# BurryChen/lv_slam

Hardware: AMD Instinct MI355X
Metric: NDT registrations/sec (64k-pt Velodyne pairs) (higher is better)
Workload: dtype f32 terms, f64 accumulation

## Files before the change

lv_slam_amd/csrc/ndt_build.hpp:

```cpp
#pragma once
#include "ndt_types.hpp"
#include "ndt_math.hpp"

__device__ __forceinline__ unsigned mm_enc_max(int ord) { return (unsigned)ord ^ 0x80000000u; }
__device__ __forceinline__ unsigned mm_enc_min(int ord) { return ~((unsigned)ord ^ 0x80000000u); }
__device__ __forceinline__ int mm_dec_max(unsigned e) { return (int)(e ^ 0x80000000u); }
__device__ __forceinline__ int mm_dec_min(unsigned e) { return (int)(~e ^ 0x80000000u); }

#define MM_ILP 3
struct __attribute__((packed, aligned(4))) MmQuad { float v[4]; };
__global__ void __launch_bounds__(256) k_minmax(const float* __restrict__ tgt, size_t pitch, const int* __restrict__ cnt, unsigned* mm) {
  const int b = blockIdx.y;
  const int n = cnt[b];
  const float* X = tgt + (size_t)b * 3 * pitch;
  int mn[3] = {INT_MAX, INT_MAX, INT_MAX}, mx[3] = {INT_MIN, INT_MIN, INT_MIN};
  auto take = [&](const float x, const float y, const float z) {
    if (!finite3(x, y, z)) return;
    const int ox = f2ord(x), oy = f2ord(y), oz = f2ord(z);
    mn[0] = min(mn[0], ox); mx[0] = max(mx[0], ox);
    mn[1] = min(mn[1], oy); mx[1] = max(mx[1], oy);
    mn[2] = min(mn[2], oz); mx[2] = max(mx[2], oz);
  };
  const int stride = (int)(gridDim.x * blockDim.x) * 4;
  for (int i0 = (int)(blockIdx.x * blockDim.x + threadIdx.x) * 4; i0 < n; i0 += stride * MM_ILP) {
// ... 158 lines not shown
  const int nw = gd[b].nwords;
  const int lane = threadIdx.x & 63, wv = threadIdx.x >> 6;
  unsigned base = 0;
  for (int w0 = 0; w0 < nw; w0 += RANK_THREADS * RANK_ROWS) {
    const int wbase = w0 + wv * 64 * RANK_ROWS;
    unsigned c[RANK_ROWS], ex[RANK_ROWS], run = 0;
#pragma unroll
    for (int u = 0; u < RANK_ROWS; u++) { const int w = wbase + u * 64 + lane; c[u] = (w < nw) ? (unsigned)__popcll(W[w].bits) : 0u; }
#pragma unroll
    for (int u = 0; u < RANK_ROWS; u++) {
      unsigned inc = c[u];
#pragma unroll
      for (int o = 1; o < 64; o <<= 1) { const unsigned t = __shfl_up(inc, o); if (lane >= o) inc += t; }
      ex[u] = run + inc - c[u];
      run += __shfl(inc, 63);
    }
    if (lane == 0) wtot[wv] = run;
    __syncthreads();
    if (wv == 0) {
      const unsigned v = lane < RANK_WAVES ? wtot[lane] : 0u;
      unsigned inc = v;
#pragma unroll
      for (int o = 1; o < RANK_WAVES; o <<= 1) { const unsigned t = __shfl_up(inc, o); if (lane >= o) inc += t; }
      if (lane < RANK_WAVES) wtot[lane] = inc - v;
      if (lane == RANK_WAVES - 1) wtot[16] = inc;
    }
    __syncthreads();
    const unsigned off = base + wtot[wv];
#pragma unroll
    for (int u = 0; u < RANK_ROWS; u++) { const int w = wbase + u * 64 + lane; if (w < nw) W[w].prefix = off + ex[u]; }
    base += wtot[16];
    __syncthreads();
  }
  if (threadIdx.x == 0) gd[b].n_voxels = (int)base;
  unsigned hbase = 0;
  for (unsigned q0 = 0; q0 < n_slices; q0 += RANK_THREADS) {
    const unsigned q = q0 + threadIdx.x;
    const unsigned c = q < n_slices ? head_cnt[(size_t)b * n_slices + q] : 0u;
    unsigned tot;
    const unsigned ex = block_exscan<RANK_THREADS>(c, &tot, wtot);
    const unsigned* H = heads + ((size_t)b * n_slices + q) * slice_cap;
    unsigned* S = seg_start + gd[b].rec_off + hbase + ex;
    for (unsigned k = 0; k < c; k++) S[k] = H[k];
    hbase += tot;
  }
}

__global__ void __launch_bounds__(256) k_sorted_points(const float* __restrict__ tgt, size_t pitch, const unsigned* __restrict__ vals, float4* __restrict__ sorted,
                                                        int nx, int n_targets) {
  int b, bx;
  if (!xcd_map(nx, n_targets, bx, b)) return;
  const float* X = tgt + (size_t)b * 3 * pitch;
  const unsigned* V = vals + (size_t)b * pitch;
  float4* P = sorted + (size_t)b * pitch;
  const size_t i0 = ((size_t)bx * 256 + threadIdx.x);
  const size_t stride = (size_t)nx * 256;
  for (size_t i = i0; i < pitch; i += stride * RUN_ILP) {
    unsigned v[RUN_ILP];
    float4 q[RUN_ILP];
#pragma unroll
    for (int u = 0; u < RUN_ILP; u++) { const size_t j = i + u * stride; v[u] = j < pitch ? V[j] : 0u; }
#pragma unroll
    for (int u = 0; u < RUN_ILP; u++) { const unsigned k = v[u] < pitch ? v[u] : 0u; q[u] = make_float4(X[k], X[pitch + k], X[2 * pitch + k], 0.f); }
#pragma unroll
    for (int u = 0; u < RUN_ILP; u++) { const size_t j = i + u * stride; if (j < pitch) P[j] = q[u]; }
  }
}

#ifdef NDT_TIMELINE
__device__ unsigned long long g_ltl[16];
#define LTL_DECL unsigned long long ltl[12] = {0, 0, 0, 0, 0, 0, 0, 0, 0, 0, 0, 0}; unsigned long long ltl_last = __builtin_readcyclecounter(); const unsigned long long ltl_t0 = ltl_last
#define LTL_STAMP(k) do { __builtin_amdgcn_sched_barrier(0); const unsigned long long t_ = __builtin_readcyclecounter(); ltl[k] += t_ - ltl_last; ltl_last = t_; __builtin_amdgcn_sched_barrier(0); } while (0)
#define LTL_COUNT(k, v) do { ltl[k] += (unsigned long long)(v); } while (0)
#define LTL_FLUSH() do { ltl[10] = 1; ltl[11] = __builtin_readcyclecounter() - ltl_t0; if ((threadIdx.x & 63) == 0 && (blockIdx.x % 24) == (threadIdx.x >> 6) * 5) for (int k_ = 0; k_ < 12; k_++) atomicAdd(&g_ltl[k_], ltl[k_]); } while (0)
#define LTL_ARRIVED1(a) asm volatile("" : "+v"(a))
#else
#define LTL_DECL do {} while (0)
#define LTL_STAMP(k) do {} while (0)
#define LTL_COUNT(k, v) do {} while (0)
#define LTL_FLUSH() do {} while (0)
#define LTL_ARRIVED1(a) do {} while (0)
#endif
#define LS_WAVES 4
template <typename KeyT, bool CENT, bool SORTED = false>
__global__ void __launch_bounds__(64 * LS_WAVES) k_leafsum(const float* __restrict__ tgt, size_t pitch,
                                                           const KeyT* __restrict__ keys, const unsigned* __restrict__ vals ,
                                                           const GridDesc* __restrict__ gd, const unsigned* __restrict__ seg_start,
                                                           double* sums, int* vox_idx, int* vox_n, int cb, float* cent,
                                                           int nx, int n_targets) {
  __shared__ double term[LS_WAVES][64][9];
  __shared__ float termf[CENT ? LS_WAVES : 1][64][3];
  int b, bx;
  if (!xcd_map(nx, n_targets, bx, b)) return;
  const GridDesc& g = gd[b];
  const int lane = threadIdx.x & 63, wv = threadIdx.x >> 6;
  const KeyT* K = keys + (size_t)b * pitch;
  const unsigned* V = vals + (size_t)b * pitch;
  const float* X = tgt + (size_t)b * 3 * pitch;
  const int id0 = bx * LS_WAVES + wv, idstep = nx * LS_WAVES;
  size_t start_next = id0 < g.n_voxels ? seg_start[g.rec_off + id0] : 0;
  LTL_DECL;
  for (int id = id0; id < g.n_voxels; id += idstep) {
    LTL_COUNT(9, 1);
    const size_t start = start_next;
    if (id + idstep < g.n_voxels) start_next = seg_start[g.rec_off + id + idstep];
    double acc = (lane == 3 || lane == 6 || lane == 8) ? 1.0 : 0.0;
    float accf = 0.f;
    int cnt = 0;
    KeyT key = 0;
    for (size_t j0 = start;; j0 += 64) {
      const size_t j = j0 + lane;
      const bool inb = j < pitch;
      const KeyT kj = inb ? K[j] : (KeyT)0;
      float4 pj = make_float4(0.f, 0.f, 0.f, 0.f);
      unsigned pi = 0u;
      if (SORTED) { if (inb) pj = reinterpret_cast<const float4*>(vals)[(size_t)b * pitch + j]; }
      else pi = inb ? V[j] : 0u;
#ifdef NDT_TIMELINE
      { KeyT kq = kj; LTL_ARRIVED1(kq); LTL_ARRIVED1(pi); LTL_ARRIVED1(pj.x); }
      LTL_STAMP(0);
      LTL_COUNT(8, 1);
#endif
      if (j0 == start) key = __shfl(kj, 0);
      const bool in = inb && kj == key;
      const int m = (int)__popcll(__ballot(in));
      if (in) {
        float fx = SORTED ? pj.x : X[pi], fy = SORTED ? pj.y : X[pitch + pi], fz = SORTED ? pj.z : X[2 * pitch + pi];
        LTL_ARRIVED1(fx); LTL_ARRIVED1(fy); LTL_ARRIVED1(fz);
        LTL_STAMP(1);
        const double x = (double)fx, y = (double)fy, z = (double)fz;
        double* t = term[wv][lane];
        t[0] = x; t[1] = y; t[2] = z;
        t[3] = x * x; t[4] = x * y; t[5] = x * z; t[6] = y * y; t[7] = y * z; t[8] = z * z;
        if (CENT) { termf[wv][lane][0] = fx; termf[wv][lane][1] = fy; termf[wv][lane][2] = fz; }
      }
      __builtin_amdgcn_wave_barrier();
      LTL_STAMP(2);
      if (lane < 9) {
        int l = 0;
        for (; l + 8 <= m; l += 8) {
          double t[8];
#pragma unroll
          for (int u = 0; u < 8; u++) t[u] = term[wv][l + u][lane];
#pragma unroll
          for (int u = 0; u < 8; u++) acc += t[u];
        }
        for (; l < m; l++) acc += term[wv][l][lane];
      } else if (CENT && lane < 12) {
        for (int l = 0; l < m; l++) accf += termf[wv][l][lane - 9];
      }
      __builtin_amdgcn_wave_barrier();
      LTL_STAMP(3);
      cnt += m;
      if (m < 64) break;
    }
    if (lane < 9) sums[(size_t)(g.rec_off + id) * 9 + lane] = acc;
    else if (CENT && lane < 12) cent[(size_t)(g.rec_off + id) * 3 + (lane - 9)] = accf / (float)cnt;
    if (lane == 0) {
      vox_idx[g.rec_off + id] = (int)((unsigned)key & ((1u << cb) - 1u));
      vox_n[g.rec_off + id] = cnt;
    }
    LTL_STAMP(4);
  }
  LTL_FLUSH();
}

#ifndef LS_TREE_LEAVES
#define LS_TREE_LEAVES 1
#endif
__global__ void __launch_bounds__(64 * LS_WAVES) k_leafsum_tree(const float* __restrict__ tgt, size_t pitch, const unsigned* __restrict__ keys, const unsigned* __restrict__ vals,
                                                                const GridDesc* __restrict__ gd, const unsigned* __restrict__ seg_start,
                                                                double* sums, int* vox_idx, int* vox_n, int cb, int nx, int n_targets) {
  int b, bx;
  if (!xcd_map(nx, n_targets, bx, b)) return;
  const GridDesc& g = gd[b];
  const int lane = threadIdx.x & 63, wv = threadIdx.x >> 6;
  const unsigned* K = keys + (size_t)b * pitch;
  const unsigned* V = vals + (size_t)b * pitch;
  const float* X = tgt + (size_t)b * 3 * pitch;
  constexpr int NL = LS_TREE_LEAVES;
  const int id0 = bx * LS_WAVES + wv, idstep = nx * LS_WAVES;
  const int nv = g.n_voxels;
  for (int idb = id0; idb < nv; idb += NL * idstep) {
    size_t start[NL];
    bool have[NL];
#pragma unroll
    for (int u = 0; u < NL; u++) { const int id = idb + u * idstep; have[u] = id < nv; start[u] = have[u] ? seg_start[g.rec_off + id] : 0; }
    double a[NL][9];
    int cnt[NL];
    unsigned key[NL];
    bool more[NL];
#pragma unroll
    for (int u = 0; u < NL; u++) {
#pragma unroll
      for (int k = 0; k < 9; k++) a[u][k] = 0.0;
      cnt[u] = 0; key[u] = 0u; more[u] = have[u];
    }
    for (int chunk = 0;; chunk++) {
      bool any = false;
#pragma unroll
      for (int u = 0; u < NL; u++) any = any || more[u];
      if (!any) break;
      unsigned kj[NL], pi[NL];
      bool inb[NL];
#pragma unroll
      for (int u = 0; u < NL; u++) {
        const size_t j = start[u] + (size_t)chunk * 64 + lane;
        inb[u] = more[u] && j < pitch;
        kj[u] = inb[u] ? K[j] : 0u;
        pi[u] = inb[u] ? V[j] : 0u;
      }
      float fx[NL], fy[NL], fz[NL];
      bool in[NL];
#pragma unroll
      for (int u = 0; u < NL; u++) {
        if (chunk == 0) key[u] = __shfl(kj[u], 0);
        in[u] = inb[u] && kj[u] == key[u];
        fx[u] = fy[u] = fz[u] = 0.f;
        if (in[u]) { fx[u] = X[pi[u]]; fy[u] = X[pitch + pi[u]]; fz[u] = X[2 * pitch + pi[u]]; }
      }
#pragma unroll
      for (int u = 0; u < NL; u++) {
        const int m = (int)__popcll(__ballot(in[u]));
        if (in[u]) {
          const double x = (double)fx[u], y = (double)fy[u], z = (double)fz[u];
          a[u][0] += x; a[u][1] += y; a[u][2] += z;
          a[u][3] += x * x; a[u][4] += x * y; a[u][5] += x * z; a[u][6] += y * y; a[u][7] += y * z; a[u][8] += z * z;
        }
        cnt[u] += m;
        more[u] = more[u] && m == 64;
      }
    }
    typedef unsigned int u2v __attribute__((ext_vector_type(2)));
#pragma unroll
    for (int u = 0; u < NL; u++) {
      if (!have[u]) continue;
      const int id = idb + u * idstep;
      double p1[5], p2[3];
#pragma unroll
      for (int i = 0; i < 5; i++) {
        const double x = a[u][i], v = (i + 5 < 9) ? a[u][i + 5] : 0.0;
        const u2v lo = __builtin_amdgcn_permlane32_swap((unsigned)__double2loint(x), (unsigned)__double2loint(v), false, false);
        const u2v hi = __builtin_amdgcn_permlane32_swap((unsigned)__double2hiint(x), (unsigned)__double2hiint(v), false, false);
        p1[i] = __hiloint2double((int)hi.x, (int)lo.x) + __hiloint2double((int)hi.y, (int)lo.y);
      }
#pragma unroll
      for (int i = 0; i < 3; i++) {
        const double x = p1[i], v = (i + 3 < 5) ? p1[i + 3] : 0.0;
        const u2v lo = __builtin_amdgcn_permlane16_swap((unsigned)__double2loint(x), (unsigned)__double2loint(v), false, false);
        const u2v hi = __builtin_amdgcn_permlane16_swap((unsigned)__double2hiint(x), (unsigned)__double2hiint(v), false, false);
        double w = __hiloint2double((int)hi.x, (int)lo.x) + __hiloint2double((int)hi.y, (int)lo.y);
#pragma unroll
        for (int o = 8; o > 0; o >>= 1) w += __shfl_xor(w, o);
        p2[i] = w;
      }
      if ((lane & 15) == 0) {
        const int row = lane >> 4, base = 3 * (row & 1) + 5 * (row >> 1), nrow = (row & 1) ? ((row >> 1) ? 1 : 2) : 3;
        double* o = sums + (size_t)(g.rec_off + id) * 9;
#pragma unroll
        for (int i = 0; i < 3; i++) if (i < nrow) { const int k = base + i; o[k] = p2[i] + ((k == 3 || k == 6 || k == 8) ? 1.0 : 0.0); }
      }
      if (lane == 0) {
        vox_idx[g.rec_off + id] = (int)(key[u] & ((1u << cb) - 1u));
        vox_n[g.rec_off + id] = cnt[u];
      }
    }
  }
}

__global__ void __launch_bounds__(256) k_voxels(const GridDesc* __restrict__ gd, const double* __restrict__ sums,
                                                 VoxelRec* recs, int* vox_n, double eig_mult, int pca, double* icov64, int* kd_weight,
                                                 VoxelRecF* recs_fast ) {
  const int b = blockIdx.y;
  const GridDesc& g = gd[b];
  const int id = blockIdx.x * blockDim.x + threadIdx.x;
  if (id >= g.n_voxels) return;
  const double* A = sums + (size_t)(g.rec_off + id) * 9;
  const double S[3] = {A[0], A[1], A[2]};
  const double C[9] = {A[3], A[4], A[5], A[4], A[6], A[7], A[5], A[7], A[8]};
  const int cnt = vox_n[g.rec_off + id];
  const double dn = (double)cnt;
  double mu[3] = {S[0] / dn, S[1] / dn, S[2] / dn};
  double cov[9];
  for (int a = 0; a < 3; a++)
    for (int c = 0; c < 3; c++) cov[a * 3 + c] = (C[a * 3 + c] - 2 * (S[a] * mu[c])) / dn + mu[a] * mu[c];
  const double f = (dn - 1.0) / dn;
  for (int a = 0; a < 9; a++) cov[a] *= f;
  double ev[3], Vm[9];
  ndtm::eigen_sym3(cov, ev, Vm);
  VoxelRec r;
  r.mean[0] = mu[0]; r.mean[1] = mu[1]; r.mean[2] = mu[2];
  for (int a = 0; a < 9; a++) r.icov[a] = 0.f;
  r.weight = 1;
  int n_out = cnt, kd_w = 0;
  if (ev[0] < 0 || ev[1] < 0 || ev[2] <= 0) {
    n_out = -1;
    r.weight = VOX_DEAD;
    if (icov64) for (int a = 0; a < 9; a++) icov64[(size_t)(g.rec_off + id) * 9 + a] = 0.0;
  } else {
    const double minev = eig_mult * ev[2];
    if (ev[0] < minev) {
      ev[0] = minev;
      if (ev[1] < minev) ev[1] = minev;
      double VD[9], Vi[9];
      for (int a = 0; a < 3; a++) for (int c = 0; c < 3; c++) VD[a * 3 + c] = Vm[a * 3 + c] * ev[c];
      ndtm::mat3_inverse(Vm, Vi);
      ndtm::mat3_mul(VD, Vi, cov);
    }
    if (pca) {
      double s0 = sqrt(ev[0]), s1 = sqrt(ev[1]), s2 = sqrt(ev[2]);
      double f0 = (s2 - s1) / s2, f1 = (s1 - s0) / s2, f2 = s0 / s2;
      int label = 1;
      double fm = f0;
      if (f1 > fm) { fm = f1; label = 2; }
      if (f2 > fm) { label = 3; }
      double scale = (label == 2) ? 1.25 : ((label == 1) ? 0.75 : 1.0);
      double d2d = scale * sqrt((mu[0] * mu[0] + mu[1] * mu[1]) + mu[2] * mu[2]);
      r.weight = (int)d2d;
      kd_w = r.weight;
    }
    double ic[9];
    ndtm::mat3_inverse(cov, ic);
    bool bad = false;
    for (int a = 0; a < 9; a++) { if (!isfinite(ic[a])) bad = true; r.icov[a] = (float)ic[a]; }
    if (bad) { n_out = -1; r.weight = VOX_DEAD; }
    if (icov64) for (int a = 0; a < 9; a++) icov64[(size_t)(g.rec_off + id) * 9 + a] = ic[a];
  }
  recs[g.rec_off + id] = r;
  vox_n[g.rec_off + id] = n_out;
  if (recs_fast) {
    VoxelRecF f;
    for (int a = 0; a < 3; a++) { f.mh[a] = (float)r.mean[a]; f.ml[a] = (float)(r.mean[a] - (double)f.mh[a]); }
    f.c[0] = r.icov[0]; f.c[1] = 0.5f * (r.icov[1] + r.icov[3]); f.c[2] = 0.5f * (r.icov[2] + r.icov[6]);
    f.c[3] = r.icov[4]; f.c[4] = 0.5f * (r.icov[5] + r.icov[7]); f.c[5] = r.icov[8];
    f.pad_[0] = f.pad_[1] = f.pad_[2] = 0.f;
    f.weight = r.weight;
    recs_fast[g.rec_off + id] = f;
  }
  if (kd_weight) kd_weight[g.rec_off + id] = kd_w;
}
```

lv_slam_amd/csrc/ndt_engine.hpp:

```cpp
#pragma once

struct mi355ndt_handle;
struct EngineDel { void operator()(mi355ndt_handle* e) const { (void)mi355ndt_destroy(e); } };

struct StreamCtx {
  long long batch_id = -1; int n_pairs = 0;
  bool busy = false;
  bool redo = false;
  bool done_sync = false;
  long long launch = -1;
  DevBuf<int> d_in; PinBuf<int> h_in; unsigned* h_in_dev = nullptr;
  PinBuf<mi355ndt_result> h_res; mi355ndt_result* d_res_map = nullptr;
  std::vector<float> guesses;
  PoseRecord* d_pose = nullptr; int pose_cap = 0, pose_base = 0, pose_stride = 1;
  std::unique_ptr<mi355ndt_handle, EngineDel> e;
};
struct StreamState {
  static constexpr int EV = 16;
  bool sync_only = false, drop_carry = true;
  int nctx = 0, max_pairs = 0, items = 0, ring_cap = 0, thresh = 0;
  bool thresh_given = false;
  size_t max_tgt = 0, max_src = 0;
  int plan_cb = 0; size_t plan_words = 0;
  void* pose_next = nullptr; size_t pose_cap_next = 0; int pose_base_next = 0, pose_stride_next = 1;
  long long next_id = 0, launches = 0, counted = 0;
  long long recovered_upto = -1;
  DevBuf<AsyncCtl> d_ctl;
  DevBuf<int> d_ring;
  DevBuf<CtxStat> d_stat;
  HipStream build_stream; int reserve_wg = 0, launch_slots = 0;
  bool lean = false;
  bool reserve_given = false;
  int last_reserve = 0, last_slots = 0;
  HipEvent ev_built[ASYNC_MAX_CTX], ev_launched[EV], ev_prepared[EV]; bool prep_first = true;
  PinBuf<volatile StreamStatus> h_status; StreamStatus* d_status = nullptr;
  StreamCtx ctx[ASYNC_MAX_CTX];
};

struct VoxelScratch {
  DevBuf<float> in, x, out;
  DevBuf<unsigned char> keep;
  DevBuf<unsigned> keys, vals;
  DevBuf<unsigned> hist, offs, tmp;
  DevBuf<int> flag, pos;
  DevBuf<int> mm, cnt, aabb, stat;
  DevBuf<PfGrid> grid; DevBuf<McBox> box;
  DevBuf<unsigned char> tab; PinBuf<unsigned char> h_tab;
  DevBuf<double> part; PinBuf<double> h_part;
  PinBuf<int> h_ret;
  bool pending = false;
};

struct CloudIndex {
  static constexpr int NO_INDEX = -1;
  DevBuf<unsigned char> blob; int status = NO_INDEX; int n_fin = 0;
};

struct GicpCache {
  DevBuf<double> cov;
  int k = -1; double eps = 0.0;
};
struct GicpSide {
  DevBuf<float> rows_own; size_t n = 0, pitch = 0;
  int kf_id = -1; bool set = false;
  CloudIndex index; GicpCache cache;
};

struct mi355ndt_handle {
  int device = 0;
  HipStream own_stream;
  hipStream_t stream = nullptr;
  mi355ndt_params prm;
  std::string err;

  int n_pairs = 0, cap_pairs = 0;
  size_t tgt_pitch = 0, src_pitch = 0;
  size_t own_tgt_pitch = 0, own_src_pitch = 0;
  int own_tgt_pairs = 0, own_src_pairs = 0;
  DevBuf<float> d_tgt_own, d_src_own;
  const float *d_tgt = nullptr, *d_src = nullptr;
  DevBuf<int> d_tgt_cnt_own, d_src_cnt_own;
  int *d_tgt_cnt = nullptr, *d_src_cnt = nullptr;
  std::vector<int> h_tgt_cnt, h_src_cnt;
  std::vector<int> up_tgt_cnt, up_src_cnt;
  bool have_target = false, have_source = false;
  GridsBuilt built{};
  bool aligned_once = false;

  unsigned* d_minmax = nullptr;
  DevBuf<GridDesc> d_grid;
  DevBuf<unsigned> d_nwords, d_word_off;
  DevBuf<unsigned> d_keys_a, d_keys_b;
  DevBuf<unsigned> d_vals_a, d_vals_b;
  DevBuf<BitWord> d_words;
  size_t recs_per_pair = 0;
  DevBuf<VoxelRec> d_recs; DevBuf<int> d_vox_idx, d_vox_n;
  DevBuf<unsigned> d_seg_start; DevBuf<double> d_sums;
  DevBuf<unsigned> d_heads, d_head_cnt;
  DevBuf<float> d_cent; DevBuf<double> d_icov64;
  DevBuf<int> d_kdw;
  DevBuf<float4> d_sorted; bool leaf_sorted = false;
  DevBuf<unsigned> d_rs_hist, d_rs_offs;
  DevBuf<double> d_fit;
  DevBuf<BitWord> d_fwords; DevBuf<unsigned> d_fruns;
  DevBuf<int> d_fit_items; DevBuf<float> d_fit_T;
  DevBuf<float> d_pf_out; int pf_count = 0; size_t pf_pitch = 0;
  CloudIndex ol_index; DevBuf<float> d_ol_dist; PinBuf<float> h_ol_dist;
  int ol_cell_mm = 100;
  int pf_group = 0;
  VoxelScratch vs;
  struct Keyframe {
    DevBuf<float> rows; size_t n = 0, pitch = 0; int ch = 3;
    CloudIndex index;
    GicpCache gicp;
  };
  std::map<int, Keyframe> keyframes;
  int kf_next_id = 0;
  int kff_cell_mm = 100;
  struct Gicp {
    mi355ndt_gicp_params prm{20, 1e-3, 2e-3, 5e-4, 200, 20, 5.0};
    GicpSide side[2];
    DevBuf<int> idx, m; DevBuf<double> maha, part; DevBuf<float> moved;
    PinBuf<double> h_rec; double* d_rec = nullptr;
    bool have_corr = false, have_final = false; int n_matched = 0;
    float final_cm[16] = {1,0,0,0, 0,1,0,0, 0,0,1,0, 0,0,0,1};
  } gicp;
  struct GicpBatch {
    struct Slot {
      GicpSide side;
      DevBuf<int> idx; DevBuf<double> maha, part;
      bool have_final = false; float final_cm[16];
    };
    std::vector<Slot> slot;
    DevBuf<int> m;
    PinBuf<double> h_rec; double* d_rec = nullptr;
    PinBuf<GcSlot> h_tab; DevBuf<GcSlot> d_tab;
    int rounds = 0; std::vector<int> requests;
  } gicp_batch;
  struct IcpWork {
    DevBuf<float> W, d2; DevBuf<int> idx; DevBuf<double> part;
    size_t n = 0, pitch = 0;
    bool have_final = false; IcpRun run;
  };
  struct Icp {
    mi355ndt_icp_params prm{0.0, 10, -DBL_MAX, 1.3407807929942596e154, 3, 0};
    GicpSide side[2];
    IcpWork work;
    DevBuf<int> m; DevBuf<float> moved;
    PinBuf<double> h_rec; double* d_rec = nullptr;
  } icp;
  struct IcpBatch {
    struct Slot { GicpSide side; IcpWork work; };
    std::vector<Slot> slot;
    DevBuf<int> m;
    PinBuf<double> h_rec; double* d_rec = nullptr;
    PinBuf<IcpSlot> h_tab; DevBuf<IcpSlot> d_tab;
    int rounds = 0; std::vector<int> requests;
  } icp_batch;
  float last_final[16] = {1,0,0,0, 0,1,0,0, 0,0,1,0, 0,0,0,1};
  PinBuf<unsigned> h_pin_u;

  DevBuf<PairState> d_state;
  DevBuf<double> d_partials;
  int chunks_per_pair = 0;
  int rows_per_pair = 0, pts_per_chunk = CHUNK_PTS;
  int items_per_pair = 0;
  bool async_force = false;
  bool async_align = true;
  int score_only_last = 1;
  DevBuf<int> d_ring; DevBuf<unsigned> d_arrived; DevBuf<AsyncCtl> d_actl;
  PinBuf<AsyncCtl> h_pin_actl;
  DevBuf<AsyncTab> d_atab;
  unsigned debug_abort_pos = 0xFFFFFFFFu;
  unsigned debug_ring_mask = 0xFFu;
  int sweep_waves = 0;
  int last_async_wpe = 0, last_async_grid = 0;
  int arith = 0;
  DevBuf<VoxelRecF> d_recs_fast;
  int pose_model = 0;
  int ndt_class = 0;
  DevBuf<double> d_pcl_rows;
  DevBuf<float> d_euler_rows;
  int f32_sum_order = 0;
  double gauss_last[3] = {0, 0, 0};
// ... 144 lines not shown
```

lv_slam_amd/csrc/ndt_host_build.hpp:

```cpp
#pragma once

static int build_targets_impl(mi355ndt_handle* h, const GridExtras make) {
  if (h->n_pairs <= 0 || !h->d_tgt) return MI355NDT_ERR_STATE;
  HIPCHK(h, hipSetDevice(h->device));
  { int rcu = uploads_before_compute(h); if (rcu) return rcu; }
  const int B = h->n_pairs;
  const size_t pitch = h->tgt_pitch;
  const size_t total = (size_t)B * pitch;
  hipStream_t s = h->stream;
  if (h->async_build && h->counts_preloaded) {
    h->up_tgt_cnt.clear();
  } else if (h->up_tgt_cnt.size() != (size_t)B || !std::equal(h->up_tgt_cnt.begin(), h->up_tgt_cnt.end(), h->h_tgt_cnt.begin())) {
    HIPCHK(h, hipMemcpyAsync(h->d_tgt_cnt, h->h_tgt_cnt.data(), B * sizeof(int), hipMemcpyHostToDevice, s));
    HIPCHK(h, hipStreamSynchronize(s));
    h->up_tgt_cnt.assign(h->h_tgt_cnt.begin(), h->h_tgt_cnt.begin() + B);
  }

  HIPCHK(h, h->d_keys_a.reserve(total)); HIPCHK(h, h->d_keys_b.reserve(total));
  HIPCHK(h, h->d_vals_a.reserve(total)); HIPCHK(h, h->d_vals_b.reserve(total));
  const int minpts = h->prm.min_points_per_voxel;
  const size_t rpp = pitch / (size_t)minpts + 1;
  if (rpp > ((size_t)1 << ID_BITS)) { h->err = "target too large: voxel ids would not fit the sweep's queue entries"; return MI355NDT_ERR_BAD_ARG; }
  if ((size_t)B * rpp > h->d_recs.cap || rpp != h->recs_per_pair) {
    const size_t need = (size_t)B * rpp;
    h->recs_per_pair = 0;
    HIPCHK(h, h->d_recs.realloc_exact(need)); HIPCHK(h, h->d_vox_idx.realloc_exact(need)); HIPCHK(h, h->d_vox_n.realloc_exact(need));
    HIPCHK(h, h->d_seg_start.realloc_exact(need)); HIPCHK(h, h->d_sums.realloc_exact(need * 9)); HIPCHK(h, h->d_cent.realloc_exact(need * 3));
    h->recs_per_pair = rpp;
  }
  h->ev_last_fresh = false;
  const bool build_events = h->prof && !(h->build_stamped && h->async_build);
  if (build_events) HIPCHK(h, ev_begin(h, h->ev_build));
  const int gx = (int)((pitch + 255) / 256);
  h->built.valid = false;
  if (!h->word_off_cleared) HIPCHK(h, hipMemsetAsync(h->d_word_off, 0, (2 + 6 * (size_t)h->cap_pairs) * sizeof(unsigned), s));
  h->word_off_cleared = false;
  k_minmax<<<dim3(std::max(1, std::min((gx + 3) / 4 / MM_ILP, 64)), B), 256, 0, s>>>(h->d_tgt, pitch, h->d_tgt_cnt, h->d_minmax);
  k_griddesc<<<(B + 63) / 64, 64, 0, s>>>(h->d_minmax, h->d_grid, h->d_nwords, h->prm.resolution, B, (unsigned)rpp);
  k_word_offsets<<<1, 1024, 0, s>>>(h->d_grid, h->d_nwords, B, h->d_word_off);
  size_t total_words;
  int cb;
  const bool planned = h->async_build && h->plan_cb > 0 && h->plan_words > 0 && h->plan_words <= h->d_words.cap && h->d_bstat;
  if (planned) {
    k_build_check<<<(B + 255) / 256, 256, 0, s>>>(h->d_word_off, h->d_grid, h->d_nwords, B, (unsigned)std::min(h->plan_words, (size_t)0xFFFFFFFFu), h->plan_cb, h->d_bstat + 1);
    total_words = h->plan_words;
    cb = h->plan_cb;
  } else {
    HIPCHK(h, hipMemcpyAsync(h->h_pin_u, h->d_word_off, 2 * sizeof(unsigned), hipMemcpyDeviceToHost, s));
    HIPCHK(h, hipStreamSynchronize(s));
    total_words = h->h_pin_u[0];
    cb = std::max(1, ceil_log2(h->h_pin_u[1] + 1u));
    if (h->async_build) cb = std::max(cb, h->plan_cb);
    if (h->d_bstat) HIPCHK(h, hipMemsetAsync(h->d_bstat + 3, 0, sizeof(unsigned), s));
  }
  if (total_words > h->d_words.cap) HIPCHK(h, h->d_words.reserve(std::max(total_words, (size_t)1024)));
  if (total_words) HIPCHK(h, hipMemsetAsync(h->d_words, 0, total_words * sizeof(BitWord), s));
  const bool want_cent = make.cent, fast_recs = make.recs_fast, want_kdw = make.kdw;
  if (make.icov64) HIPCHK(h, h->d_icov64.reserve(h->d_recs.cap * 9));
  if (fast_recs) HIPCHK(h, h->d_recs_fast.reserve(h->d_recs.cap));
  if (want_kdw) HIPCHK(h, h->d_kdw.reserve(h->d_recs.cap));
  {
    unsigned *ka = h->d_keys_a, *kb = h->d_keys_b;
    const RsPlan plan = rs_plan(cb);
    const int npass = plan.passes;
    const int tiles = (int)((pitch + RS_TILE - 1) / RS_TILE);
    const size_t rs_need = ((size_t)B * tiles) << RS_MAX_BITS;
    HIPCHK(h, h->d_rs_hist.reserve(rs_need)); HIPCHK(h, h->d_rs_offs.reserve(rs_need));
    unsigned *kin = (npass & 1) ? ka : kb, *kout = (npass & 1) ? kb : ka;
    unsigned *vin = (npass & 1) ? h->d_vals_a : h->d_vals_b, *vout = (npass & 1) ? h->d_vals_b : h->d_vals_a;
    const RsPoints points = {h->d_tgt, h->d_tgt_cnt, h->d_grid, cb, kin};
    if (!rs_disjoint(kin, vin, kout, vout, total)) { h->err = "target build: the sort's two buffer pairs overlap"; return MI355NDT_ERR_STATE; }
    for (int p = 0; p < npass; p++) {
      rs_pass(s, plan.bits, kin, vin, kout, vout, pitch, p * plan.bits, h->d_rs_hist, h->d_rs_offs, tiles, B, p == 0, p == 0 ? &points : nullptr);
      std::swap(kin, kout); std::swap(vin, vout);
    }
    const unsigned nsl = ls_slices(pitch), scap = ls_slice_cap(minpts);
    HIPCHK(h, h->d_heads.reserve((size_t)B * nsl * scap));
    HIPCHK(h, h->d_head_cnt.reserve((size_t)B * nsl));
    k_mark<unsigned><<<dim3((nsl + 3) / 4, B), 256, 0, s>>>(kb, pitch, h->d_grid, h->d_words, h->d_heads, h->d_head_cnt, nsl, scap, minpts, cb);
    k_rank<<<B, RANK_THREADS, 0, s>>>(h->d_grid, h->d_words, h->d_heads, h->d_head_cnt, nsl, scap, h->d_seg_start);
    const int lb = std::max(1, std::min((int)((rpp + LS_WAVES - 1) / LS_WAVES), 64));
    auto leafsum = [&](auto kern, const unsigned* vals) {
      kern<<<xcd_grid(lb, B), 64 * LS_WAVES, 0, s>>>(h->d_tgt, pitch, kb, vals, h->d_grid, h->d_seg_start, h->d_sums, h->d_vox_idx, h->d_vox_n, cb, h->d_cent, lb, B);
    };
    if (fast_recs && !want_cent && !h->leaf_sorted) {
      k_leafsum_tree<<<xcd_grid(lb, B), 64 * LS_WAVES, 0, s>>>(h->d_tgt, pitch, kb, h->d_vals_b, h->d_grid, h->d_seg_start, h->d_sums, h->d_vox_idx, h->d_vox_n, cb, lb, B);
    } else if (h->leaf_sorted) {
      HIPCHK(h, h->d_sorted.reserve(total));
      const int gb = std::max(1, std::min((int)((pitch + 256 * RUN_ILP - 1) / (256 * RUN_ILP)), 64));
      k_sorted_points<<<xcd_grid(gb, B), 256, 0, s>>>(h->d_tgt, pitch, h->d_vals_b, h->d_sorted, gb, B);
      leafsum(want_cent ? k_leafsum<unsigned, true, true> : k_leafsum<unsigned, false, true>, reinterpret_cast<const unsigned*>(h->d_sorted.p));
    } else leafsum(want_cent ? k_leafsum<unsigned, true> : k_leafsum<unsigned, false>, h->d_vals_b);
  }
  k_voxels<<<dim3((unsigned)((rpp + 255) / 256), B), 256, 0, s>>>(h->d_grid, h->d_sums, h->d_recs, h->d_vox_n,
                                                                  h->prm.min_covar_eigvalue_mult, h->prm.variant == MI355NDT_VARIANT_PCA,
                                                                  make.icov64 ? h->d_icov64 : nullptr, want_kdw ? h->d_kdw : nullptr, fast_recs ? h->d_recs_fast : nullptr);
  HIPCHK(h, hipGetLastError());
  if (h->prof) {
    if (build_events) HIPCHK(h, ev_end(h, h->ev_build));
    double pts = 0;
    for (int b = 0; b < B; b++) pts += h->h_tgt_cnt[b];
    h->P.build_alg_bytes += pts * (12 + 12 + 4 + 16);
  }
  h->built = GridsBuilt{true, make, h->prm.resolution, cb, total_words, false};
  return compute_enqueued(h);
}

static int build_targets(mi355ndt_handle* h, const GridExtras make) {
  NOT_IN_STREAM(h);
  const int rc = build_targets_impl(h, make);
  if (rc != MI355NDT_OK && h->ev_compute) (void)compute_enqueued(h);
  return rc;
}
int mi355ndt_batch_build_targets(mi355ndt_handle* h) {
  if (!h) return MI355NDT_ERR_BAD_HANDLE;
  return build_targets(h, eff_extras(h));
}

static int ensure_grids(mi355ndt_handle* h, GridWant want) {
  HIPCHK(h, hipSetDevice(h->device));
  { int rcu = uploads_before_compute(h); if (rcu) return rcu; }
  const GridExtras make = eff_extras(h, want == GRIDS_LIVE);
  return grids_serve(h->built, want == GRIDS_ANY ? GridExtras{} : make) ? (int)MI355NDT_OK : build_targets(h, make);
}
```

lv_slam_amd/csrc/ndt_host_life.hpp:

```cpp
#pragma once

const char* mi355ndt_version(void) { return "mi355ndt 0.1 (gfx950)"; }

int mi355ndt_device_count(void) {
  int n = 0;
  if (hipGetDeviceCount(&n) != hipSuccess) return 0;
  return n;
}

int mi355ndt_host_numa_node(int device) {
  int node = -1;
  if (hipDeviceGetAttribute(&node, hipDeviceAttributeHostNumaId, device) != hipSuccess) {
    (void)hipGetLastError();
    char bdf[64];
    if (hipDeviceGetPCIBusId(bdf, (int)sizeof bdf, device) != hipSuccess) { (void)hipGetLastError(); return -1; }
    for (char* c = bdf; *c; c++) if (*c >= 'A' && *c <= 'F') *c = (char)(*c - 'A' + 'a');
    std::ifstream f(std::string("/sys/bus/pci/devices/") + bdf + "/numa_node");
    if (f && (f >> node)) return node;
    unsigned dom = 0, bus = 0, dv = 0, fn = 0;
    if (sscanf(bdf, "%x:%x:%x.%x", &dom, &bus, &dv, &fn) != 4) return -1;
    const long want = (long)((bus << 8) | (dv << 3) | fn);
    auto prop = [](const std::string& path, const char* key, long& out) {
      std::ifstream pf(path);
      std::string k; long v;
      while (pf >> k >> v) if (k == key) { out = v; return true; }
      return false;
    };
    const std::string top = "/sys/class/kfd/kfd/topology/nodes/";
    int gpu_node = -1;
    for (int n = 0; n < 64 && gpu_node < 0; n++) {
      long loc = -1, simd = 0;
      if (prop(top + std::to_string(n) + "/properties", "simd_count", simd) && simd > 0 &&
          prop(top + std::to_string(n) + "/properties", "location_id", loc) && loc == want) gpu_node = n;
    }
    if (gpu_node < 0) return -1;
    node = -1;
    for (int n = 0; n < 64 && node < 0; n++) {
      long cores = 0;
      if (!prop(top + std::to_string(n) + "/properties", "cpu_cores_count", cores) || cores <= 0) continue;
      for (int l = 0; l < 64; l++) {
        long to = -1;
        if (!prop(top + std::to_string(n) + "/io_links/" + std::to_string(l) + "/properties", "node_to", to)) break;
        if (to == gpu_node) { node = n; break; }
      }
    }
  }
  return node;
}

static bool numa_cpus(int node, cpu_set_t* set) {
  CPU_ZERO(set);
  if (node < 0) return false;
  std::ifstream f("/sys/devices/system/node/node" + std::to_string(node) + "/cpulist");
  std::string txt;
  if (!f || !std::getline(f, txt)) return false;
  bool any = false;
  size_t pos = 0;
  while (pos < txt.size()) {
    size_t comma = txt.find(',', pos);
    std::string part = txt.substr(pos, comma == std::string::npos ? std::string::npos : comma - pos);
    size_t dash = part.find('-');
    int lo = atoi(part.c_str()), hi = dash == std::string::npos ? lo : atoi(part.c_str() + dash + 1);
    for (int c = lo; c <= hi && c < CPU_SETSIZE; c++) { CPU_SET(c, set); any = true; }
    if (comma == std::string::npos) break;
    pos = comma + 1;
  }
  return any;
}

int mi355ndt_default_params(mi355ndt_params* p) {
  if (!p) return MI355NDT_ERR_BAD_ARG;
  p->resolution = 1.0f;
  p->step_size = 0.1;
  p->outlier_ratio = 0.55;
  p->trans_epsilon = 0.1;
  p->max_iterations = 35;
  p->neighbor_mode = MI355NDT_DIRECT7;
  p->variant = MI355NDT_VARIANT_OMP;
  p->min_points_per_voxel = 6;
  p->min_covar_eigvalue_mult = 0.01;
  return MI355NDT_OK;
}

int mi355ndt_create(const mi355ndt_params* params, int device, mi355ndt_handle** out) {
  if (!out) return MI355NDT_ERR_BAD_ARG;
  *out = nullptr;
  int n = 0;
  if (hipGetDeviceCount(&n) != hipSuccess || n <= 0) return MI355NDT_ERR_NO_DEVICE;
  if (device < 0 || device >= n) return MI355NDT_ERR_BAD_ARG;
  mi355ndt_params p;
  mi355ndt_default_params(&p);
  if (params) p = *params;
  int rc = check_params(p);
  if (rc) return rc;
  std::unique_ptr<mi355ndt_handle> h(new mi355ndt_handle());
  h->device = device;
  h->prm = p;
  gauss_constants3(0.55, 1.0f, h->gauss_last);
  { hipDeviceProp_t pr; if (hipGetDeviceProperties(&pr, device) == hipSuccess && pr.multiProcessorCount > 0) h->n_cu = pr.multiProcessorCount; }
  if (const char* e = std::getenv("MI355NDT_LEAF_SORTED")) h->leaf_sorted = std::atoi(e) != 0;
  if (const char* e = std::getenv("MI355NDT_FINE_TILES")) { const int v = std::atoi(e); if (v == 1 || v == 2) h->fine_tiles = v; }
  if (const char* e = std::getenv("MI355NDT_ARITH")) h->arith = std::atoi(e) == 1 ? 1 : 0;
  if (const char* e = std::getenv("MI355NDT_SWEEP_WAVES")) { const int v = std::atoi(e); if (v == 0 || v == 2 || v == 3) h->sweep_waves = v; }
  if (const char* e = std::getenv("MI355NDT_ASYNC")) { h->async_align = std::atoi(e) != 0; h->async_force = std::atoi(e) == 2; }
  if (const char* e = std::getenv("MI355NDT_SCORE_ONLY_LAST_SWEEP")) h->score_only_last = std::atoi(e) != 0;
  if (const char* e = std::getenv("MI355NDT_SWEEP_DYN_SHIFT")) { const int v = std::atoi(e); if (v >= 0 && v <= 30) h->dyn_shift = v; }
  if (hipSetDevice(device) != hipSuccess || h->own_stream.create() != hipSuccess) return MI355NDT_ERR_HIP;
  h->stream = h->own_stream;
  if (h->h_pin_u.realloc_exact(4) != hipSuccess ||
      h->h_pin_active.realloc_exact(128) != hipSuccess ||
      h->d_active.realloc_exact(128) != hipSuccess ||
      h->d_ctl.realloc_exact(2) != hipSuccess ||
      h->d_hits.realloc_exact(2) != hipSuccess ||
      hipMemsetAsync(h->d_hits, 0, 2 * sizeof(unsigned long long), h->stream) != hipSuccess ||
      h->d_hook.realloc_exact(64 * sizeof(double) / sizeof(float)) != hipSuccess ||
      h->ev_compute.create() != hipSuccess || h->ev_burst[0].create() != hipSuccess || h->ev_burst[1].create() != hipSuccess) return MI355NDT_ERR_HIP;
  for (int i = 0; i < mi355ndt_handle::UP_STREAMS; i++)
    if (h->copy_stream[i].create() != hipSuccess || h->ev_uploads[i].create() != hipSuccess) return MI355NDT_ERR_HIP;
  *out = h.release();
  return MI355NDT_OK;
}

int mi355ndt_destroy(mi355ndt_handle* h) {
  if (!h) return MI355NDT_ERR_BAD_HANDLE;
  (void)hipSetDevice(h->device);
  (void)hipStreamSynchronize(h->stream);
  if (h->ss) (void)mi355ndt_stream_end(h);
  for (hipStream_t cs : h->copy_stream) if (cs) (void)hipStreamSynchronize(cs);
  delete h;
  return MI355NDT_OK;
}

int mi355ndt_get_params(const mi355ndt_handle* h, mi355ndt_params* out) {
  if (!h) return MI355NDT_ERR_BAD_HANDLE;
  if (!out) return MI355NDT_ERR_BAD_ARG;
  *out = h->prm;
  return MI355NDT_OK;
}

int mi355ndt_set_stream(mi355ndt_handle* h, void* s) {
  if (!h) return MI355NDT_ERR_BAD_HANDLE;
  NOT_IN_STREAM(h);
  (void)hipSetDevice(h->device);
  (void)hipStreamSynchronize(h->stream);
  if (s) {
    h->own_stream.reset();
    h->stream = (hipStream_t)s;
  } else if (!h->own_stream) {
    HIPCHK(h, h->own_stream.create());
    h->stream = h->own_stream;
  }
  return MI355NDT_OK;
}

const char* mi355ndt_last_error(const mi355ndt_handle* h) { return h ? h->err.c_str() : "bad handle"; }

int mi355ndt_synchronize(mi355ndt_handle* h) {
  if (!h) return MI355NDT_ERR_BAD_HANDLE;
  HIPCHK(h, hipSetDevice(h->device));
  for (hipStream_t cs : h->copy_stream) if (cs) HIPCHK(h, hipStreamSynchronize(cs));
  HIPCHK(h, hipStreamSynchronize(h->stream));
  return MI355NDT_OK;
}

int mi355ndt_batch_size(const mi355ndt_handle* h) { return h ? h->n_pairs : MI355NDT_ERR_BAD_HANDLE; }

int mi355ndt_set_params(mi355ndt_handle* h, const mi355ndt_params* p) {
  if (!h) return MI355NDT_ERR_BAD_HANDLE;
  NOT_IN_STREAM(h);
  if (!p) return MI355NDT_ERR_BAD_ARG;
  int rc = check_params(*p);
  if (rc) return rc;
  const mi355ndt_params old = h->prm;
  h->prm = *p;
  const bool radius_search = class_neighbor_mode(h->ndt_class, p->neighbor_mode) == MI355NDT_KDTREE || mt_is_live(*p);
  const bool keep_grid = old.resolution != p->resolution && h->n_pairs == 1 && !h->have_source && !radius_search && h->d_tgt == h->d_tgt_own;
  const bool regrid = (old.resolution != p->resolution && !keep_grid) || old.variant != p->variant ||
                      old.min_points_per_voxel != p->min_points_per_voxel ||
                      old.min_covar_eigvalue_mult != p->min_covar_eigvalue_mult ||
                      !grids_serve(h->built, grid_extras(*p, 0, false, h->ndt_class));
  if (regrid && h->built.valid) {
    h->built.valid = false;
    rc = ensure_grids(h, GRIDS_CONFIG);
// ... 103 lines not shown
```

Before: 70750.

## Cut leaf-sum LDS footprint with half-chunk staging and prefetch next chunk

The leaf-sum kernel now packs per-lane terms into one LDS row struct and can stage a 64-point chunk through LDS in two halves, which halves shared memory per wave. It also prefetches the next chunk's keys and points during the current reduction, switches to 32-bit offsets and a scalar wave index, and uses readlane for the segment key. k_voxels parks the covariance in LDS across the eigen solve and sets a launch-bounds occupancy hint to lower register pressure. The half mode is chosen by an env var or by async_build, and a new guard rejects very large targets because of the 32-bit offsets.

```diff
diff --git a/lv_slam_amd/csrc/ndt_build.hpp b/lv_slam_amd/csrc/ndt_build.hpp
--- a/lv_slam_amd/csrc/ndt_build.hpp
+++ b/lv_slam_amd/csrc/ndt_build.hpp
@@ -264,81 +264,112 @@
 #define LTL_ARRIVED1(a) do {} while (0)
 #endif
 #define LS_WAVES 4
-template <typename KeyT, bool CENT, bool SORTED = false>
+template <bool CENT> struct LsRow { double t[9]; };
+template <> struct LsRow<true> { double t[9]; float f[4]; };
+template <typename T> __device__ __forceinline__ T ls_at(const T* base, unsigned i) {
+  return *reinterpret_cast<const T*>(reinterpret_cast<const char*>(base) + i * (unsigned)sizeof(T));
+}
+template <typename KeyT, bool CENT, bool SORTED = false, int PARTS = 1>
 __global__ void __launch_bounds__(64 * LS_WAVES) k_leafsum(const float* __restrict__ tgt, size_t pitch,
                                                            const KeyT* __restrict__ keys, const unsigned* __restrict__ vals ,
                                                            const GridDesc* __restrict__ gd, const unsigned* __restrict__ seg_start,
                                                            double* sums, int* vox_idx, int* vox_n, int cb, float* cent,
                                                            int nx, int n_targets) {
-  __shared__ double term[LS_WAVES][64][9];
-  __shared__ float termf[CENT ? LS_WAVES : 1][64][3];
+  static_assert(PARTS == 1 || PARTS == 2, "a chunk's terms pass through LDS at once or in two halves");
+  constexpr int LS_HALF = 64 / PARTS;
+  constexpr int LS_AHEAD = PARTS == 1 ? 8 : 4;
+  __shared__ LsRow<CENT> term[LS_WAVES][LS_HALF];
   int b, bx;
   if (!xcd_map(nx, n_targets, bx, b)) return;
   const GridDesc& g = gd[b];
-  const int lane = threadIdx.x & 63, wv = threadIdx.x >> 6;
+  const int lane = threadIdx.x & 63, wv = __builtin_amdgcn_readfirstlane(threadIdx.x >> 6);
   const KeyT* K = keys + (size_t)b * pitch;
   const unsigned* V = vals + (size_t)b * pitch;
-  const float* X = tgt + (size_t)b * 3 * pitch;
+  const float4* P = reinterpret_cast<const float4*>(vals) + (size_t)b * pitch;
+  const float *X = tgt + (size_t)b * 3 * pitch, *Y = X + pitch, *Z = Y + pitch;
+  const unsigned npos = (unsigned)pitch;
   const int id0 = bx * LS_WAVES + wv, idstep = nx * LS_WAVES;
-  size_t start_next = id0 < g.n_voxels ? seg_start[g.rec_off + id0] : 0;
+  unsigned start_next = id0 < g.n_voxels ? seg_start[g.rec_off + id0] : 0u;
   LTL_DECL;
   for (int id = id0; id < g.n_voxels; id += idstep) {
     LTL_COUNT(9, 1);
-    const size_t start = start_next;
+    const unsigned start = start_next;
     if (id + idstep < g.n_voxels) start_next = seg_start[g.rec_off + id + idstep];
-    double acc = (lane == 3 || lane == 6 || lane == 8) ? 1.0 : 0.0;
+    int ls = lane;
+    asm volatile("" : "+v"(ls));
+    double acc = (ls == 3 || ls == 6 || ls == 8) ? 1.0 : 0.0;
     float accf = 0.f;
     int cnt = 0;
     KeyT key = 0;
-    for (size_t j0 = start;; j0 += 64) {
-      const size_t j = j0 + lane;
-      const bool inb = j < pitch;
-      const KeyT kj = inb ? K[j] : (KeyT)0;
-      float4 pj = make_float4(0.f, 0.f, 0.f, 0.f);
-      unsigned pi = 0u;
-      if (SORTED) { if (inb) pj = reinterpret_cast<const float4*>(vals)[(size_t)b * pitch + j]; }
-      else pi = inb ? V[j] : 0u;
+    KeyT kj = 0;
+    unsigned pi = 0u;
+    float4 pj = make_float4(0.f, 0.f, 0.f, 0.f);
+    auto fetch = [&](const unsigned j) {
+      const bool inb = j < npos;
+      kj = inb ? ls_at(K, j) : (KeyT)0;
+      if (SORTED) { if (inb) pj = ls_at(P, j); }
+      else pi = inb ? ls_at(V, j) : 0u;
+    };
+    fetch(start + lane);
+    for (unsigned j0 = start;; j0 += 64) {
+      const bool inb = j0 + lane < npos;
 #ifdef NDT_TIMELINE
       { KeyT kq = kj; LTL_ARRIVED1(kq); LTL_ARRIVED1(pi); LTL_ARRIVED1(pj.x); }
       LTL_STAMP(0);
       LTL_COUNT(8, 1);
 #endif
-      if (j0 == start) key = __shfl(kj, 0);
+      if (j0 == start) key = sizeof(KeyT) == 4 ? (KeyT)__builtin_amdgcn_readlane((unsigned)kj, 0) : __shfl(kj, 0);
       const bool in = inb && kj == key;
       const int m = (int)__popcll(__ballot(in));
+      float fx = 0.f, fy = 0.f, fz = 0.f;
       if (in) {
-        float fx = SORTED ? pj.x : X[pi], fy = SORTED ? pj.y : X[pitch + pi], fz = SORTED ? pj.z : X[2 * pitch + pi];
+        fx = SORTED ? pj.x : ls_at(X, pi); fy = SORTED ? pj.y : ls_at(Y, pi); fz = SORTED ? pj.z : ls_at(Z, pi);
         LTL_ARRIVED1(fx); LTL_ARRIVED1(fy); LTL_ARRIVED1(fz);
-        LTL_STAMP(1);
-        const double x = (double)fx, y = (double)fy, z = (double)fz;
-        double* t = term[wv][lane];
-        t[0] = x; t[1] = y; t[2] = z;
-        t[3] = x * x; t[4] = x * y; t[5] = x * z; t[6] = y * y; t[7] = y * z; t[8] = z * z;
-        if (CENT) { termf[wv][lane][0] = fx; termf[wv][lane][1] = fy; termf[wv][lane][2] = fz; }
-      }
-      __builtin_amdgcn_wave_barrier();
-      LTL_STAMP(2);
-      if (lane < 9) {
-        int l = 0;
-        for (; l + 8 <= m; l += 8) {
-          double t[8];
-#pragma unroll
-          for (int u = 0; u < 8; u++) t[u] = term[wv][l + u][lane];
-#pragma unroll
-          for (int u = 0; u < 8; u++) acc += t[u];
+      }
+      if (m == 64) fetch(j0 + 64 + lane);
+      LTL_STAMP(1);
+#pragma unroll
+      for (int hf = 0; hf < PARTS; hf++) {
+        const int mh = m - hf * LS_HALF < LS_HALF ? m - hf * LS_HALF : LS_HALF;
+        if (hf && mh <= 0) break;
+        if (in && lane / LS_HALF == hf) {
+          const double x = (double)fx, y = (double)fy, z = (double)fz;
+          LsRow<CENT>& row = term[wv][lane & (LS_HALF - 1)];
+          double* t = row.t;
+          t[0] = x; t[1] = y; t[2] = z;
+          t[3] = x * x; t[4] = x * y; t[5] = x * z; t[6] = y * y; t[7] = y * z; t[8] = z * z;
+          if constexpr (CENT) { row.f[0] = fx; row.f[1] = fy; row.f[2] = fz; }
         }
-        for (; l < m; l++) acc += term[wv][l][lane];
-      } else if (CENT && lane < 12) {
-        for (int l = 0; l < m; l++) accf += termf[wv][l][lane - 9];
-      }
-      __builtin_amdgcn_wave_barrier();
-      LTL_STAMP(3);
+        __builtin_amdgcn_wave_barrier();
+        LTL_STAMP(2);
+        if (lane < 9) {
+          int l = 0;
+          for (; l + LS_AHEAD <= mh; l += LS_AHEAD) {
+            double t[LS_AHEAD];
+#pragma unroll
+            for (int u = 0; u < LS_AHEAD; u++) t[u] = term[wv][l + u].t[lane];
+#pragma unroll
+            for (int u = 0; u < LS_AHEAD; u++) acc += t[u];
+          }
+          for (; l < mh; l++) acc += term[wv][l].t[lane];
+        } else if constexpr (CENT) {
+          if (lane < 12) for (int l = 0; l < mh; l++) accf += term[wv][l].f[lane - 9];
+        }
+        __builtin_amdgcn_wave_barrier();
+        if (PARTS > 1) {
+          asm volatile("" : "+v"(fx), "+v"(fy), "+v"(fz));
+          __builtin_amdgcn_sched_barrier(0);
+        }
+        LTL_STAMP(3);
+      }
       cnt += m;
       if (m < 64) break;
     }
-    if (lane < 9) sums[(size_t)(g.rec_off + id) * 9 + lane] = acc;
-    else if (CENT && lane < 12) cent[(size_t)(g.rec_off + id) * 3 + (lane - 9)] = accf / (float)cnt;
-    if (lane == 0) {
+    ls = lane;
+    asm volatile("" : "+v"(ls));
+    if (ls < 9) sums[(size_t)(g.rec_off + id) * 9 + ls] = acc;
+    else if (CENT && ls < 12) cent[(size_t)(g.rec_off + id) * 3 + (ls - 9)] = accf / (float)cnt;
+    if (ls == 0) {
       vox_idx[g.rec_off + id] = (int)((unsigned)key & ((1u << cb) - 1u));
       vox_n[g.rec_off + id] = cnt;
     }
@@ -450,9 +481,10 @@
   }
 }
 
-__global__ void __launch_bounds__(256) k_voxels(const GridDesc* __restrict__ gd, const double* __restrict__ sums,
-                                                 VoxelRec* recs, int* vox_n, double eig_mult, int pca, double* icov64, int* kd_weight,
-                                                 VoxelRecF* recs_fast ) {
+__global__ void __launch_bounds__(256, 6) k_voxels(const GridDesc* __restrict__ gd, const double* __restrict__ sums,
+                                                    VoxelRec* recs, int* vox_n, double eig_mult, int pca, double* icov64, int* kd_weight,
+                                                    VoxelRecF* recs_fast ) {
+  __shared__ double cov_park[9][256];
   const int b = blockIdx.y;
   const GridDesc& g = gd[b];
   const int id = blockIdx.x * blockDim.x + threadIdx.x;
@@ -469,7 +501,10 @@
   const double f = (dn - 1.0) / dn;
   for (int a = 0; a < 9; a++) cov[a] *= f;
   double ev[3], Vm[9];
+  for (int a = 0; a < 9; a++) cov_park[a][threadIdx.x] = cov[a];
   ndtm::eigen_sym3(cov, ev, Vm);
+  asm volatile("" ::: "memory");
+  for (int a = 0; a < 9; a++) cov[a] = cov_park[a][threadIdx.x];
   VoxelRec r;
   r.mean[0] = mu[0]; r.mean[1] = mu[1]; r.mean[2] = mu[2];
   for (int a = 0; a < 9; a++) r.icov[a] = 0.f;
diff --git a/lv_slam_amd/csrc/ndt_engine.hpp b/lv_slam_amd/csrc/ndt_engine.hpp
--- a/lv_slam_amd/csrc/ndt_engine.hpp
+++ b/lv_slam_amd/csrc/ndt_engine.hpp
@@ -100,6 +100,7 @@
   DevBuf<float> d_cent; DevBuf<double> d_icov64;
   DevBuf<int> d_kdw;
   DevBuf<float4> d_sorted; bool leaf_sorted = false;
+  int leaf_parts = 0;
   DevBuf<unsigned> d_rs_hist, d_rs_offs;
   DevBuf<double> d_fit;
   DevBuf<BitWord> d_fwords; DevBuf<unsigned> d_fruns;
diff --git a/lv_slam_amd/csrc/ndt_host_build.hpp b/lv_slam_amd/csrc/ndt_host_build.hpp
--- a/lv_slam_amd/csrc/ndt_host_build.hpp
+++ b/lv_slam_amd/csrc/ndt_host_build.hpp
@@ -21,6 +21,7 @@
   const int minpts = h->prm.min_points_per_voxel;
   const size_t rpp = pitch / (size_t)minpts + 1;
   if (rpp > ((size_t)1 << ID_BITS)) { h->err = "target too large: voxel ids would not fit the sweep's queue entries"; return MI355NDT_ERR_BAD_ARG; }
+  if (pitch >= ((size_t)1 << 28)) { h->err = "target too large: the leaf sums address a target's rows through 32-bit byte offsets"; return MI355NDT_ERR_BAD_ARG; }
   if ((size_t)B * rpp > h->d_recs.cap || rpp != h->recs_per_pair) {
     const size_t need = (size_t)B * rpp;
     h->recs_per_pair = 0;
@@ -80,6 +81,7 @@
     k_mark<unsigned><<<dim3((nsl + 3) / 4, B), 256, 0, s>>>(kb, pitch, h->d_grid, h->d_words, h->d_heads, h->d_head_cnt, nsl, scap, minpts, cb);
     k_rank<<<B, RANK_THREADS, 0, s>>>(h->d_grid, h->d_words, h->d_heads, h->d_head_cnt, nsl, scap, h->d_seg_start);
     const int lb = std::max(1, std::min((int)((rpp + LS_WAVES - 1) / LS_WAVES), 64));
+    const bool halves = h->leaf_parts ? h->leaf_parts == 2 : h->async_build;
     auto leafsum = [&](auto kern, const unsigned* vals) {
       kern<<<xcd_grid(lb, B), 64 * LS_WAVES, 0, s>>>(h->d_tgt, pitch, kb, vals, h->d_grid, h->d_seg_start, h->d_sums, h->d_vox_idx, h->d_vox_n, cb, h->d_cent, lb, B);
     };
@@ -89,8 +91,11 @@
       HIPCHK(h, h->d_sorted.reserve(total));
       const int gb = std::max(1, std::min((int)((pitch + 256 * RUN_ILP - 1) / (256 * RUN_ILP)), 64));
       k_sorted_points<<<xcd_grid(gb, B), 256, 0, s>>>(h->d_tgt, pitch, h->d_vals_b, h->d_sorted, gb, B);
-      leafsum(want_cent ? k_leafsum<unsigned, true, true> : k_leafsum<unsigned, false, true>, reinterpret_cast<const unsigned*>(h->d_sorted.p));
-    } else leafsum(want_cent ? k_leafsum<unsigned, true> : k_leafsum<unsigned, false>, h->d_vals_b);
+      const unsigned* pts = reinterpret_cast<const unsigned*>(h->d_sorted.p);
+      if (halves) leafsum(want_cent ? k_leafsum<unsigned, true, true, 2> : k_leafsum<unsigned, false, true, 2>, pts);
+      else leafsum(want_cent ? k_leafsum<unsigned, true, true, 1> : k_leafsum<unsigned, false, true, 1>, pts);
+    } else if (halves) leafsum(want_cent ? k_leafsum<unsigned, true, false, 2> : k_leafsum<unsigned, false, false, 2>, h->d_vals_b);
+    else leafsum(want_cent ? k_leafsum<unsigned, true, false, 1> : k_leafsum<unsigned, false, false, 1>, h->d_vals_b);
   }
   k_voxels<<<dim3((unsigned)((rpp + 255) / 256), B), 256, 0, s>>>(h->d_grid, h->d_sums, h->d_recs, h->d_vox_n,
                                                                   h->prm.min_covar_eigvalue_mult, h->prm.variant == MI355NDT_VARIANT_PCA,
diff --git a/lv_slam_amd/csrc/ndt_host_life.hpp b/lv_slam_amd/csrc/ndt_host_life.hpp
--- a/lv_slam_amd/csrc/ndt_host_life.hpp
+++ b/lv_slam_amd/csrc/ndt_host_life.hpp
@@ -99,6 +99,7 @@
   gauss_constants3(0.55, 1.0f, h->gauss_last);
   { hipDeviceProp_t pr; if (hipGetDeviceProperties(&pr, device) == hipSuccess && pr.multiProcessorCount > 0) h->n_cu = pr.multiProcessorCount; }
   if (const char* e = std::getenv("MI355NDT_LEAF_SORTED")) h->leaf_sorted = std::atoi(e) != 0;
+  if (const char* e = std::getenv("MI355NDT_LEAF_PARTS")) { const int v = std::atoi(e); h->leaf_parts = (v == 1 || v == 2) ? v : 0; }
   if (const char* e = std::getenv("MI355NDT_FINE_TILES")) { const int v = std::atoi(e); if (v == 1 || v == 2) h->fine_tiles = v; }
   if (const char* e = std::getenv("MI355NDT_ARITH")) h->arith = std::atoi(e) == 1 ? 1 : 0;
   if (const char* e = std::getenv("MI355NDT_SWEEP_WAVES")) { const int v = std::atoi(e); if (v == 0 || v == 2 || v == 3) h->sweep_waves = v; }
```

After: 70870 (median of 6 runs). No clear change (+0.2%).
